# 0xC0000054/pdn-jpegxl

Hardware: AMD Instinct MI355X
Metric: megapixels/sec decode (4K lossy VarDCT) (higher is better)
Workload: dtype f32

## Files before the change

### pdn_jpegxl_amd/csrc/decoder.cc

```cpp
#include <hip/hip_runtime.h>
#include <algorithm>
#include <atomic>
#include <cmath>
#include <cstdarg>
#include <cstdio>
#include <cstdlib>
#include <cstring>
#include <memory>
#include <mutex>
#include <string>
#include <thread>
#include <vector>
#include "../../include/jxlfiletypeio.h"
#include "batch_layout.h"
#include "entropy_plan.h"
#include "host_parse.h"
#include "icc.h"
#include "kernels.h"

namespace jxlhip {

struct HipError : std::runtime_error {
  explicit HipError(const std::string& m) : std::runtime_error(m) {}
};
// ... 64 lines not shown
    std::vector<DevImage> imgs;
    std::vector<int> parse_status;
    std::vector<std::string> parse_msg;
    std::vector<size_t> status_off;
    DevImage* d_imgs = nullptr;
    bool pending = false;
    hipEvent_t lf_done = nullptr, hf_done = nullptr, done = nullptr, uploaded = nullptr;
    std::vector<Tap> taps;
    std::vector<std::string> stage_names;
    std::vector<int> stage_chain;
    std::vector<hipEvent_t> events;
    std::vector<float> stage_ms;
  };
  static constexpr int kSlots = 3;
  static constexpr int kPixelChunk = 32;
  Slot slots[kSlots];
  int cur = 0, last = 0;
  Slot* active = &slots[0];
  hipStream_t stream_lf = nullptr;
  hipStream_t stream_hf = nullptr;
  hipStream_t last_stream = nullptr;
  std::vector<std::string> total_names;
  std::vector<double> total_ms;
  int total_batches = 0;
  std::string sticky_error;
  int sticky_status = 0;
  uint8_t* li_dev = nullptr; uint8_t* li_host = nullptr; size_t li_cap = 0;
  void EnsureLoadImageBuffers(size_t bytes);
  int lane_stride_override = 0;
  int hf_stride_override = 0;
  bool debug_taps = false;
  int band_first_row = 0, band_rows = 0;
  bool no_stream_pairs = false;
  bool no_lf_pipeline = false;
  int alpha_narrow_limit = 32767;
  bool no_direct = false, mod_lanes64 = false;
  bool overlap = true;
  int downscale = 1;

  explicit JxlHipDecoder(int dev);
  ~JxlHipDecoder();
  void EnsureWs(size_t bytes);
  void EnsureBlob(size_t bytes);
  void Mark(const char* name, hipStream_t s, int chain);
  void WaitSlot(Slot& S);
  Slot& Last() { return slots[last]; }
  void Decode(int32_t n_, const uint8_t* const* host_data, const size_t* sizes, const uint8_t* const* dev_data,
              uint8_t* const* dev_out, hipStream_t stream, bool sync, DecoderStatus* statuses, ErrorInfo* err);
  DecoderStatus Finish(DecoderStatus* statuses, ErrorInfo* err);
  void CopyPlaneTap(int stage);
  void PrepassSingle(ParsedFrame& f, const uint8_t* dev_file);
  EntropyPlanOptions PlanOptions() const;
};

JxlHipDecoder::JxlHipDecoder(int dev) {
  if (dev < 0) HIP_OK(hipGetDevice(&dev));
  device = dev;
  HIP_OK(hipSetDevice(device));
  int entropy_cus = 0, pixel_cus = 0;
  if (const char* e = Knob("JXLHIP_ENTROPY_CUS")) entropy_cus = std::min(256, std::max(0, atoi(e)));
  if (const char* e = Knob("JXLHIP_PIXEL_CUS")) pixel_cus = std::min(256, std::max(0, atoi(e)));
  auto masked_stream = [](hipStream_t* s, int first, int count) {
    uint32_t mask[8] = {0, 0, 0, 0, 0, 0, 0, 0};
    for (int i = first; i < first + count; i++) mask[i >> 5] |= 1u << (i & 31);
    HIP_OK(hipExtStreamCreateWithCUMask(s, 8, mask));
  };
// ... 399 lines not shown
  if (any_alpha && !(skip_stages & 4))
    LaunchAlphaAns(d_imgs, B.alpha_tasks, nalpha_t, plan.alpha_stride, plan.alpha.Bytes(), plan.direct_alpha, plan.lean_mod,
                   alpha_narrow, s_hf);
  if (!ds || any_alpha) Mark("alpha_ans", s_hf, 1);
  if (debug_taps && !ds) {
    taps.assign(n, Tap());
    LaunchExpandCoefficients(d_imgs, n, true, B.max_tiles, stream);
    HIP_OK(hipStreamSynchronize(stream));
    CopyPlaneTap(0);
  }
  const bool finish_on_hf = s_hf == stream || debug_taps || !Knob("JXLHIP_ALPHA_FINISH_ON_PIX");
  if (finish_on_hf) {
    if (any_alpha && !(skip_stages & 4)) LaunchAlphaFinish(d_imgs, n, max_groups, alpha_narrow > 0, s_hf);
    if (!ds || any_alpha) Mark("alpha_finish", s_hf, 1);
  }
  if (s_hf != stream) {
    HIP_OK(hipEventRecord(S.hf_done, s_hf));
    HIP_OK(hipStreamWaitEvent(stream, S.hf_done, 0));
  }
  Mark("main_start", stream, 2);
  if (!finish_on_hf) {
    if (any_alpha && !(skip_stages & 4)) LaunchAlphaFinish(d_imgs, n, max_groups, alpha_narrow > 0, stream);
    Mark("alpha_finish", stream, 2);
  }
  hipStream_t s_pix = pix_on_hf ? s_hf : stream;
  if (ds && B.any_vardct) {
    if (any_alpha) LaunchAlphaReduce(d_imgs, n, B.max_ds_cells, s_pix);
    LaunchLfOutput(d_imgs, n, B.max_ds_cells, s_pix);
    Mark("lf_output", s_pix, 2);
  }
  for (int c0 = 0; c0 < (ds ? 0 : n); c0 += pixel_chunk) {
    const int cnt = std::min(pixel_chunk, n - c0);
    if (!(skip_stages & 8))
    LaunchReconTiles(d_imgs + c0, cnt, B.max_tiles, d_basis_all, d_basis_small, d_llf_scale, d_basis_mfma, s_pix);
    Mark("reconstruct", s_pix, 2);
    LaunchExpandCoefficients(d_imgs + c0, cnt, false, B.max_tiles, s_pix);
    LaunchGenericReconstruct(d_imgs + c0, cnt, d_basis_all, d_basis_small, d_llf_scale, s_pix);
    Mark("reconstruct_generic", s_pix, 2);
    if (debug_taps) { HIP_OK(hipStreamSynchronize(s_pix)); CopyPlaneTap(1); }
    if (any_noise && !(early_noise && c0 == 0)) { LaunchNoise(d_imgs + c0, cnt, max_groups, B.max_w, B.max_h, s_pix); Mark("noise", s_pix, 2); }
    if (!(skip_stages & 16))
    LaunchFilterTiles(d_imgs + c0, cnt, B.max_w, B.max_h, B.stage_mask, B.any_unfiltered, B.any_fused, B.any_fused2, s_pix);
    Mark("filters+output", s_pix, 2);
  }
  if (s_pix != stream) {
    HIP_OK(hipEventRecord(S.hf_done, s_pix));
    HIP_OK(hipStreamWaitEvent(stream, S.hf_done, 0));
  }
  if (nmod_t) {
    if (s_lf != stream) { HIP_OK(hipEventRecord(S.lf_done, s_lf)); HIP_OK(hipStreamWaitEvent(stream, S.lf_done, 0)); }
    LaunchModularAns(d_imgs, n, B.mod_tasks, nmod_t, plan.mod.Bytes(), plan.max_mod_groups,
                     plan.max_mod_coded, plan.mod_lanes, plan.mod_rb, plan.mod_wp_lds, plan.direct_mod, stream);
    for (auto& op : B.mod_ops) {
      if (op.kind == 3) LaunchModularPalette(op.a, op.b, op.out, op.nout, op.type, op.rw, op.rh, op.status, stream);
      else LaunchModularOp(op.kind, op.a, op.b, op.c, op.aw, op.ah, op.rw, op.rh, op.type, stream);
    }
    LaunchModularOut(d_imgs, n, B.max_mod_pixels, stream);
    if (ds) LaunchBoxReduce(d_imgs, n, B.max_ds_cells, stream);
    Mark("modular", stream, 2);
  }
  if (!patches.tiles.empty()) {
    LaunchPatches(B.patch_frames, B.patch_tiles, (int)patches.tiles.size(), B.patch_list, B.patch_pos, B.patch_refs, stream);
    Mark("patches", stream, 2);
  }
  if (!comps.empty()) {
    LaunchCompose(B.comp_imgs, B.comp_frames, (int)comps.size(), B.max_segments, stream);
    Mark("compose", stream, 2);
// ... 203 lines not shown
    return DecoderStatus_DecodeError;
  }
}

DecoderStatus jxlhip_finish(JxlHipDecoder* dec, DecoderStatus* statuses, ErrorInfo* err) {
  if (!dec) return DecoderStatus_NullParameter;
  try {
    return dec->Finish(statuses, err);
  } catch (const std::exception& e) {
    SetErr(err, "%s", e.what());
    return DecoderStatus_DecodeError;
  }
}

int32_t jxlhip_set_option(JxlHipDecoder* dec, const char* name, int32_t value) {
  if (!dec || !name) return 0;
  if (!strcmp(name, "debug_taps")) { dec->debug_taps = value != 0; return 1; }
  if (!strcmp(name, "query_pixel_chunk")) return JxlHipDecoder::kPixelChunk;
  if (!strcmp(name, "lane_stride")) { if (value != 0 && !PowerOfTwoUpTo64(value)) return 0; dec->lane_stride_override = value; return 1; }
  if (!strcmp(name, "band_first_row")) { if (value < 0) return 0; dec->band_first_row = value; return 1; }
  if (!strcmp(name, "band_rows")) { if (value < 0) return 0; dec->band_rows = value; return 1; }
  if (!strcmp(name, "no_direct")) { dec->no_direct = value != 0; return 1; }
  if (!strcmp(name, "alpha_narrow_limit")) { if (value < 0 || value > 32767) return 0; dec->alpha_narrow_limit = value; return 1; }
  if (!strcmp(name, "query_alpha_narrow_groups") || !strcmp(name, "query_alpha_redo_groups")) {
    JxlHipDecoder::Slot& S = dec->Last();
    if (S.pending || !S.h_status) return -1;
    const int word = name[12] == 'n' ? kStatusAlphaNarrow : kStatusAlphaRedo;
    int64_t sum = 0;
    for (int i = 0; i < S.n; i++) sum += S.h_status[(size_t)i * 16 + word];
    return (int32_t)std::min<int64_t>(sum, INT32_MAX);
  }
  if (!strcmp(name, "no_stream_pairs")) { dec->no_stream_pairs = value != 0; return 1; }
  if (!strcmp(name, "no_lf_pipeline")) { dec->no_lf_pipeline = value != 0; return 1; }
  if (!strcmp(name, "mod_lanes64")) { dec->mod_lanes64 = value != 0; return 1; }
  if (!strcmp(name, "overlap")) { dec->overlap = value != 0; return 1; }
  if (!strcmp(name, "downscale")) { if (value != 1 && value != 8) return 0; dec->downscale = value; return 1; }
  return 0;
}

size_t jxlhip_read_plane(JxlHipDecoder* dec, int32_t index, const char* name, int32_t channel, void* dst, size_t capacity) {
  if (!dec || !name) return 0;
  JxlHipDecoder::Slot& S = dec->Last();
  if (index < 0 || index >= S.n || S.pending) return 0;
  if (S.parse_status[index] != DecoderStatus_Ok) return 0;
  const DevImage& d = S.imgs[index];
  std::string nm(name);
  const size_t cells = (size_t)d.w8 * d.h8, pix = (size_t)d.wp * d.hp;
  const void* src = nullptr;
  size_t bytes = 0;
  bool host = false;
  const int c = std::min(2, std::max(0, channel));
  if (nm == "lf") { src = d.lf_final[c]; bytes = cells * 4; }
  else if (nm == "lf_quant") { src = d.lfq[c]; bytes = cells * 4; }
  else if (nm == "cellinfo") { src = d.cellinfo; bytes = cells * 4; }
  else if (nm == "raw_quant") { src = d.rawq; bytes = cells * 2; }
  else if (nm == "sharpness") { src = d.sharp; bytes = cells; }
  else if (nm == "ytox") { src = d.ytox; bytes = (size_t)d.wt * d.ht; }
  else if (nm == "ytob") { src = d.ytob; bytes = (size_t)d.wt * d.ht; }
  else if (nm == "alpha") { src = d.alpha; bytes = (size_t)d.w * d.h; }
  else if (nm == "inv_sigma") { src = d.inv_sigma; bytes = cells * 4; }
  else if (dec->debug_taps && (size_t)index < S.taps.size()) {
    host = true;
    if (nm == "qcoef") { src = S.taps[index].qcoef[c].data(); bytes = S.taps[index].qcoef[c].size(); }
    else if (nm == "xyb_idct") { src = S.taps[index].xyb_idct[c].data(); bytes = S.taps[index].xyb_idct[c].size(); }
    else if (nm == "xyb_filtered") { src = S.taps[index].xyb_filtered[c].data(); bytes = S.taps[index].xyb_filtered[c].size(); }
    else if (nm == "noise_rnd") { src = S.taps[index].noise_rnd[c].data(); bytes = S.taps[index].noise_rnd[c].size(); }
// ... 230 lines not shown
```

### pdn_jpegxl_amd/csrc/kernels.h

```cpp
#pragma once
#include <hip/hip_runtime.h>
#include "dev_types.h"

namespace jxlhip {

void LaunchLfAns(const DevImage* imgs, const SectionTask* tasks, int ntasks, int slots, size_t lds_bytes, int scalar_rows, bool lean, hipStream_t s);
void LaunchLfFinish(const DevImage* imgs, const SectionTask* tasks, int ntasks, bool pipeline, hipStream_t s);
void LaunchHfBlockList(const DevImage* imgs, int nimg, int max_groups, hipStream_t s);
void LaunchHfDecode(const DevImage* imgs, const SectionTask* tasks, int nwg, int threads, int lane_stride, size_t lds_bytes, size_t lane_bytes,
                    hipStream_t s);
void LaunchAlphaAns(const DevImage* imgs, const SectionTask* tasks, int nwg, int lane_stride, size_t lds_bytes, int scalar_rows, bool lean, int narrow_limit,
                    hipStream_t s);
void LaunchAlphaFinish(const DevImage* imgs, int nimg, int max_groups, bool narrow, hipStream_t s);
void LaunchModularAns(const DevImage* imgs, int nimg, const SectionTask* tasks, int ntasks, size_t lds_bytes, int max_sections, int max_coded,
                      int lanes, int rb_width, int wp_lds, int scalar_rows, hipStream_t s);
void LaunchModularOp(int kind, int32_t* a, int32_t* b, int32_t* c, int aw, int ah, int rw, int rh, int type, hipStream_t s);
void LaunchModularPalette(const int32_t* palette, const int32_t* index, int32_t* const* out, int nout, int nb_colors, int w, int h, uint32_t* status,
                          hipStream_t s);
void LaunchModularOut(const DevImage* imgs, int nimg, size_t max_pixels, hipStream_t s);
void LaunchOrient(const uint8_t* src, uint8_t* dst, int w, int h, int px_bytes, int orientation, hipStream_t s);
void LaunchLfPixelStages(const DevImage* imgs, int nimg, size_t max_cells, hipStream_t s);
void LaunchExpandCoefficients(const DevImage* imgs, int nimg, bool all_tiles, int max_tiles, hipStream_t s);
void LaunchGenericReconstruct(const DevImage* imgs, int nimg, const float* basis_all, const float* basis_small,
                              const float* llf_scale, hipStream_t s);
void LaunchReconTiles(const DevImage* imgs, int nimg, int max_tiles, const float* basis_all, const float* basis_small,
                      const float* llf_scale, const float* basis_mfma, hipStream_t s);
void LaunchFilterTiles(const DevImage* imgs, int nimg, int max_w, int max_h, int stage_mask, bool any_unfiltered,
                       int any_fused, int any_fused2, hipStream_t s);

void LaunchLfOutput(const DevImage* imgs, int nimg, size_t max_cells, hipStream_t s);
void LaunchAlphaReduce(const DevImage* imgs, int nimg, size_t max_cells, hipStream_t s);
void LaunchBoxReduce(const DevImage* imgs, int nimg, size_t max_cells, hipStream_t s);

void LaunchNoise(const DevImage* imgs, int nimg, int max_groups, int max_w, int max_h, hipStream_t s);

void LaunchCompose(const ComposeImage* imgs, const ComposeFrame* frames, int nimg, int max_segments, hipStream_t s);
void LaunchPatches(const PatchFrame* frames, const PatchTile* tiles, int ntiles, const int32_t* list, const PatchPos* pos, const PatchRef* refs,
                   hipStream_t s);

void LaunchStatusToHost(const uint32_t* src, uint32_t* dst_pinned, int nwords, hipStream_t s);
#ifdef JXLHIP_EXPERIMENTS
void LaunchInterference(int kind, int wg_per_cu, int lds_kb, float ms, float* scratch, size_t scratch_bytes, hipStream_t s);
#endif

}
```

### pdn_jpegxl_amd/csrc/tile_kernels.hip

```cpp
#include <hip/hip_runtime.h>
#include <cstdlib>
#include "dev_types.h"
#include "dev_util.h"
#include "kernels.h"

namespace jxlhip {

#ifndef JXLHIP_PRIO_PIXEL
#define JXLHIP_PRIO_PIXEL 0
#endif
#if JXLHIP_PRIO_PIXEL
#define JXL_PIXEL_PRIO() __builtin_amdgcn_s_setprio(JXLHIP_PRIO_PIXEL)
#else
#define JXL_PIXEL_PRIO() ((void)0)
#endif

namespace {

constexpr int kTS = 64;
constexpr int kLP = 65;

__device__ const uint8_t t_quant_table[kNumStrategies] = {0, 1, 2, 3, 4, 5, 6, 6, 7, 7, 8, 8, 9, 9, 10, 10, 10, 10, 11, 12, 12, 13, 14, 14, 15, 16, 16};

__device__ __forceinline__ bool Special(uint32_t s) { return (s >= 1 && s <= 3) || (s >= 12 && s <= 17); }
typedef float __attribute__((ext_vector_type(4))) F4;
template <int N>
__device__ __forceinline__ F4 MfmaChain(const float* pa, int sa, const float* pb, int sb) {
  float a[N / 4], b[N / 4];
#pragma unroll
  for (int k = 0; k < N / 4; k++) { a[k] = pa[k * sa]; b[k] = pb[k * sb]; }
  F4 acc = {0.f, 0.f, 0.f, 0.f};
#pragma unroll
  for (int k = 0; k < N / 4; k++) acc = __builtin_amdgcn_mfma_f32_16x16x4f32(a[k], b[k], acc, 0, 0, 0);
  return acc;
}
template <bool kTableIsA>
__device__ __forceinline__ F4 MfmaChain32L(const float4* t_lo, const float4* t_hi, int pair, const float* po, int so) {
  const float4 v0 = t_lo[pair], v1 = t_hi[pair];
  const float t[8] = {v0.x, v0.y, v0.z, v0.w, v1.x, v1.y, v1.z, v1.w};
  float o[8];
#pragma unroll
  for (int k = 0; k < 8; k++) o[k] = po[k * so];
  F4 acc = {0.f, 0.f, 0.f, 0.f};
#pragma unroll
  for (int k = 0; k < 8; k++)
    acc = kTableIsA ? __builtin_amdgcn_mfma_f32_16x16x4f32(t[k], o[k], acc, 0, 0, 0) : __builtin_amdgcn_mfma_f32_16x16x4f32(o[k], t[k], acc, 0, 0, 0);
  return acc;
}
template <bool kTableIsA>
__device__ __forceinline__ F4 MfmaChain64L(const float4* t64, int pair, const float* po, int so) {
  float t[16], o[16];
#pragma unroll
  for (int j = 0; j < 4; j++) {
    const float4 v = t64[j * 256 + pair];
    t[4 * j] = v.x; t[4 * j + 1] = v.y; t[4 * j + 2] = v.z; t[4 * j + 3] = v.w;
  }
#pragma unroll
  for (int k = 0; k < 16; k++) o[k] = po[k * so];
  F4 acc = {0.f, 0.f, 0.f, 0.f};
#pragma unroll
  for (int k = 0; k < 16; k++)
    acc = kTableIsA ? __builtin_amdgcn_mfma_f32_16x16x4f32(t[k], o[k], acc, 0, 0, 0) : __builtin_amdgcn_mfma_f32_16x16x4f32(o[k], t[k], acc, 0, 0, 0);
  return acc;
}
__device__ __forceinline__ bool MfmaRows(uint32_t tl, uint32_t tr) {
  return (tl >> 31) && (tr >> 31) && ((tl >> 21) & 7) >= 1 && ((tl >> 21) & 7) == ((tr >> 21) & 7) && ((tl >> 13) & 31) == ((tr >> 13) & 31);
}
__device__ __forceinline__ bool MfmaCols(uint32_t tl, uint32_t bl) {
  return (tl >> 31) && (bl >> 31) && ((tl >> 18) & 7) >= 1 && ((tl >> 18) & 7) == ((bl >> 18) & 7) && ((tl >> 8) & 31) == ((bl >> 8) & 31);
}

__device__ __forceinline__ float SrgbOetfT(float v) {
  const float lin = 12.92f * v;
  const float cur = 1.055f * __builtin_amdgcn_exp2f(__builtin_amdgcn_logf(v) * (1.0f / 2.4f)) - 0.055f;
  return v <= 0.0031308f ? lin : cur;
}
__device__ __forceinline__ float SrgbOetf255T(float v) {
  const float lin = (12.92f * 255.0f) * v;
  const float cur = (1.055f * 255.0f) * __builtin_amdgcn_exp2f(__builtin_amdgcn_logf(v) * (1.0f / 2.4f)) - (0.055f * 255.0f);
  return v <= 0.0031308f ? lin : cur;
}
__device__ __forceinline__ float PowT(float a, float e) { return __builtin_amdgcn_exp2f(__builtin_amdgcn_logf(a) * e); }
__device__ __forceinline__ float EncodeTransferT(int kind, float v, float pq_scale, const float* lut = nullptr) {
  if (kind == 0) return v;
  if (kind == 5) {
    const float t = __builtin_sqrtf(fminf(fmaxf(v, 0.f), 1.f)) * 4095.0f;
    const int i = min((int)t, 4094);
    return lut[i] + (lut[i + 1] - lut[i]) * (t - (float)i);
  }
  const float a = fabsf(v);
  float r;
  if (kind == 1) r = a <= 0.0031308f ? 12.92f * a : 1.055f * PowT(a, 1.0f / 2.4f) - 0.055f;
  else if (kind == 2) r = a < 0.018f ? 4.5f * a : 1.099f * PowT(a, 0.45f) - 0.099f;
  else {
    const float xp = a > 0.f ? PowT(a * pq_scale, 0.1593017578125f) : 0.f;
    r = a > 0.f ? PowT((0.8359375f + 18.8515625f * xp) / (1.0f + 18.6875f * xp), 78.84375f) : 0.f;
  }
// ... 103 lines not shown
  }
  WritePixelA(im, x, y, X, Y, B, a);
}
__device__ __forceinline__ void WritePixel(const DevImage& im, int x, int y, float X, float Y, float B) {
  const uint32_t a = im.has_alpha ? LoadAlpha(im, (size_t)y * im.w + x) : 0u;
  if (im.has_noise) { WritePixelGeneral(im, x, y, X, Y, B, a); return; }
  WritePixelA(im, x, y, X, Y, B, a);
}

}

#define JXL_IDCT_STEP(Bp, v0, v1)                                                                  \
  {                                                                                                \
    const float4 b0 = *(const float4*)(Bp);                                                        \
    const float4 b1 = *(const float4*)((Bp) + 4);                                                  \
    a0[0] += v0 * b0.x; a0[1] += v0 * b0.y; a0[2] += v0 * b0.z; a0[3] += v0 * b0.w;                \
    a0[4] += v0 * b1.x; a0[5] += v0 * b1.y; a0[6] += v0 * b1.z; a0[7] += v0 * b1.w;                \
    a1[0] += v1 * b0.x; a1[1] += v1 * b0.y; a1[2] += v1 * b0.z; a1[3] += v1 * b0.w;                \
    a1[4] += v1 * b1.x; a1[5] += v1 * b1.y; a1[6] += v1 * b1.z; a1[7] += v1 * b1.w;                \
  }

__device__ __forceinline__ float DequantBias(int32_t v, float qb, float qb3) {
  if (v == 0) return 0.f;
  if (v == 1) return qb;
  if (v == -1) return -qb;
  const float f = (float)v;
  return f - qb3 * __builtin_amdgcn_rcpf(f);
}
typedef int __attribute__((ext_vector_type(4))) I4v;

constexpr int kTileF = kTS * kLP;

__global__ __launch_bounds__(768, 6) void recon_tile_kernel(const DevImage* __restrict__ imgs, const float* basis_all, const float* basis_small,
                                                             const float* llf_scale, const float* basis_mfma) {
  JXL_PIXEL_PRIO();
  extern __shared__ __align__(16) uint8_t smem_raw[];
  float* cfc3 = (float*)smem_raw;
  float* B816 = cfc3 + 3 * kTileF;
  float* cscale = B816 + 320;
  uint32_t* ci = (uint32_t*)(cscale + 64);
  uint32_t* cmeta = ci + 64;
  uint32_t* cnq = cmeta + 64;
  uint32_t* cpre = cnq + 64;
  uint32_t* cstart = cpre + 3 * 64;
  uint32_t* ctot = cstart + 3 * 64;
  const U32x2** csc = (const U32x2**)(ctot + 4);
  float4* t32_lo = (float4*)(csc + 64);
  float4* t32_hi = t32_lo + 128;
  float4* t64 = t32_hi + 128;
  const DevImage& im = imgs[blockIdx.y];
  const int tile = blockIdx.x;
  if (tile >= im.wt * im.ht) return;
  const int tid = threadIdx.x;
  const int tx = tile % im.wt, ty = tile / im.wt;
  if (ty < im.dec_gy0 * 4 || ty >= im.dec_gy1 * 4) return;
  const int wave = tid >> 6, lane = tid & 63, team = wave >> 2, tw = wave & 3;
  const int c = team == 0 ? 1 : (team == 1 ? 0 : 2);
  const int wp = im.wp, hp = im.hp;
  {
    float4* z = (float4*)cfc3;
    for (int i = tid; i < 3 * kTileF / 4; i += 768) z[i] = make_float4(0.f, 0.f, 0.f, 0.f);
  }
  int bad = 0, has64 = 0;
  if (tid < 64) {
    const int cx = tx * 8 + (tid & 7), cy = ty * 8 + (tid >> 3);
    const bool inside = cx < im.w8 && cy < im.h8;
    const size_t cell_g = (size_t)min(cy, im.h8 - 1) * im.w8 + min(cx, im.w8 - 1);
    const size_t ncells = (size_t)im.w8 * im.h8;
    const uint32_t info_g = im.cellinfo[cell_g];
    const uint32_t rq_g = im.rawq[cell_g];
    U32x2 blk[3];
    blk[0] = im.cblk[ncells + cell_g]; blk[1] = im.cblk[cell_g]; blk[2] = im.cblk[2 * ncells + cell_g];
    const uint32_t info = inside ? info_g : 0u;
    const uint32_t rqv = inside ? rq_g : 1u;
    const int ix = (info >> 8) & 31, iy = (info >> 13) & 31, lcx = (info >> 18) & 7, lcy = (info >> 21) & 7;
    if (inside) {
      if (!(info >> 31)) bad = 1;
      else {
        const int ox = (tid & 7) - ix, oy = (tid >> 3) - iy;
        bad = ox < 0 || oy < 0 || ox + (1 << lcx) > 8 || oy + (1 << lcy) > 8 || Special(info & 0xFF) ||
              (ox & ((1 << lcx) - 1)) != 0 || (oy & ((1 << lcy) - 1)) != 0;
      }
    }
    const bool valid = (info >> 31) && !bad;
    has64 = valid && (lcx == 3 || lcy == 3);
    {
      const uint64_t any = __ballot(has64);
      if (tid == 0) ctot[3] = any != 0;
    }
    const uint32_t q = t_quant_table[valid ? (info & 0xFF) : 0];
    const uint32_t rq_origin = (uint32_t)__shfl((int)rqv, valid ? tid - iy * 8 - ix : tid);
    const uint32_t lng = 3 + max(lcx, lcy);
    const bool transposed = lcy >= lcx;
    ci[tid] = info;
    cscale[tid] = im.inv_global_scale / (float)rq_origin;
    cmeta[tid] = lng | (transposed ? 16u : 0u);
    cnq[tid] = im.dq_n[q];
    csc[tid] = im.scan[q];
    const bool origin = valid && ix == 0 && iy == 0;
    uint32_t cnt[3], sum[3];
#pragma unroll
    for (int t = 0; t < 3; t++) {
      cnt[t] = origin ? blk[t].y : 0u;
      if (cnt[t] > 65536u || blk[t].x > kGroupEntriesCap - cnt[t]) cnt[t] = 0;
      sum[t] = cnt[t];
    }
#pragma unroll
    for (int d = 1; d < 64; d <<= 1) {
#pragma unroll
      for (int t = 0; t < 3; t++) {
        const uint32_t a = (uint32_t)__shfl_up((int)sum[t], d);
        if (tid >= d) sum[t] += a;
      }
    }
#pragma unroll
    for (int t = 0; t < 3; t++) {
      cpre[t * 64 + tid] = sum[t] - cnt[t];
      cstart[t * 64 + tid] = blk[t].x;
      if (tid == 63) ctot[t] = sum[t];
    }
  } else if (tid < 64 + 320) {
    B816[tid - 64] = basis_all[tid - 64];
  } else if (tid < 64 + 320 + 256) {
    const int i = tid - (64 + 320);
    const float4 v = ((const float4*)basis_mfma)[i];
    if (i & 1) t32_hi[i >> 1] = v; else t32_lo[i >> 1] = v;
  }
  if (im.num_passes > 1) bad = 1;
  if (__syncthreads_or(bad)) {
    if (tid == 0) im.tile_list[atomicAdd(&im.status[1], 1u)] = (uint32_t)tile;
    return;
  }
  if (ctot[3]) {
    for (int i = tid; i < 1024; i += 768) t64[(i & 3) * 256 + (i >> 2)] = ((const float4*)(basis_mfma + 1024))[i];
  }
  const float* const Bl = basis_all;
  float* const cfc = cfc3 + team * kTileF;
  if (tw == 0) {
    const int cxg = tx * 8 + (lane & 7), cyg = ty * 8 + (lane >> 3);
    const bool inside = cxg < im.w8 && cyg < im.h8;
    const float lf_g = im.lf_final[c][(size_t)min(cyg, im.h8 - 1) * im.w8 + min(cxg, im.w8 - 1)];
    const float lfv = inside ? lf_g : 0.f;
    const uint32_t info = ci[lane];
    const bool valid = info >> 31;
    const int ix = (info >> 8) & 31, iy = (info >> 13) & 31, lcx = (info >> 18) & 7, lcy = (info >> 21) & 7;
    const int cx = 1 << lcx, cy = 1 << lcy;
    const int ox = (lane & 7) - ix, oy = (lane >> 3) - iy;
    const float* Bx = basis_small + (cx * cx - 1) / 3 + ix * cx;
    const float* By = basis_small + (cy * cy - 1) / 3 + iy * cy;
    float bx[8], byv[8];
#pragma unroll
// ... 11 lines not shown
      const float v = __shfl(row, ((oy + k) * 8 + (lane & 7)) & 63);
      if (valid && k < cy) acc += v * byv[k];
    }
    if (valid) atomicAdd(&cfc[(oy * 8 + iy) * kLP + ox * 8 + ix], acc * sc);
  }
  {
    const size_t tile_cfl = (size_t)ty * im.wt + tx;
    const float cfl_x = im.base_x + (float)im.ytox[tile_cfl] * im.inv_color_factor;
    const float cfl_b = im.base_b + (float)im.ytob[tile_cfl] * im.inv_color_factor;
    const uint32_t* entries = im.centries + (size_t)((ty >> 2) * im.xg + (tx >> 2) - im.centries_g0) * kGroupEntriesCap;
    const uint32_t t0 = ctot[0], t01 = t0 + ctot[1], total = t01 + ctot[2];
    const float qb3 = im.qbias[3];
    for (uint32_t e = (uint32_t)tid; e < total; e += 768) {
      const uint32_t t = (e >= t0) + (e >= t01);
      const uint32_t el = e - (t == 0 ? 0u : (t == 1 ? t0 : t01));
      const uint32_t* pre = cpre + t * 64;
      uint32_t j = 0;
#pragma unroll
      for (int step = 32; step; step >>= 1) if (pre[j + step] <= el) j += step;
      const uint32_t ent = entries[cstart[t * 64 + j] + (el - pre[j])];
      const uint32_t k = ent & 0xFFFFu, nq = cnq[j];
      if (k >= nq) continue;
      const int chan = t == 0 ? 1 : (t == 1 ? 0 : 2);
      const U32x2 se = csc[j][(size_t)chan * nq + k];
      const uint32_t meta = cmeta[j];
      const uint32_t lng = meta & 15, p = se.x;
      const uint32_t r = p >> lng, cc = p & ((1u << lng) - 1);
      const uint32_t ky = (meta & 16) ? cc : r, kx = (meta & 16) ? r : cc;
      if (ky >= 64 || kx >= 64) continue;
      const int32_t v = (int32_t)ent >> 16;
      const float dm = t == 0 ? 1.0f : (t == 1 ? im.x_dm : im.b_dm);
      const float o = DequantBias(v, im.qbias[chan], qb3) * (cscale[j] * dm) * __uint_as_float(se.y);
      const uint32_t at = ((j >> 3) * 8 + ky) * kLP + (j & 7) * 8 + kx;
      atomicAdd(&cfc3[t * kTileF + at], o);
      if (t == 0) {
        if (cfl_x != 0.f) atomicAdd(&cfc3[kTileF + at], o * cfl_x);
        if (cfl_b != 0.f) atomicAdd(&cfc3[2 * kTileF + at], o * cfl_b);
      }
    }
  }
  __syncthreads();
  const int l16 = tid & 15, lq = lane >> 4;
  {
    F4 acc[4];
    bool m[4];
    const int x0 = tw * 16;
#pragma unroll
    for (int rb = 0; rb < 4; rb++) {
      const uint32_t inf = ci[rb * 16 + tw * 2];
      m[rb] = MfmaRows(inf, ci[rb * 16 + tw * 2 + 1]);
      if (m[rb]) {
        const int iy = (inf >> 13) & 31, lcy = (inf >> 21) & 7, R = 8 << lcy;
        const float* cp = cfc + ((rb * 2 - iy) * 8 + lq) * kLP + x0 + l16;
        if (R == 16) acc[rb] = MfmaChain<16>(B816 + 64 + lq * 16 + iy * 8 + l16, 64, cp, 4 * kLP);
        else if (R == 32) acc[rb] = MfmaChain32L<true>(t32_lo, t32_hi, (iy * 8 + l16) * 4 + lq, cp, 4 * kLP);
        else acc[rb] = MfmaChain64L<true>(t64, (iy * 8 + l16) * 4 + lq, cp, 4 * kLP);
      }
    }
    const int x = x0 + (lane & 7) * 2, cr = lane >> 3;
    const uint32_t info = ci[cr * 8 + (x >> 3)];
    const bool valu = (info >> 31) && !MfmaRows(ci[(cr >> 1) * 16 + (x >> 4) * 2], ci[(cr >> 1) * 16 + (x >> 4) * 2 + 1]);
    float a0[8] = {0, 0, 0, 0, 0, 0, 0, 0}, a1[8] = {0, 0, 0, 0, 0, 0, 0, 0};
    if (valu) {
      const int iy = (info >> 13) & 31, lcy = (info >> 21) & 7;
      const int R = 8 << lcy;
      const float* in = cfc + (cr - iy) * 8 * kLP + x;
      if (R == 8) {
#pragma unroll 2
        for (int k = 0; k < 8; k++) { const float v0 = in[k * kLP], v1 = in[k * kLP + 1]; JXL_IDCT_STEP(B816 + k * 8, v0, v1) }
      } else if (R == 16) {
        const float* B = B816 + 64 + iy * 8;
#pragma unroll 2
        for (int k = 0; k < 16; k++) { const float v0 = in[k * kLP], v1 = in[k * kLP + 1]; JXL_IDCT_STEP(B + k * 16, v0, v1) }
      } else {
        const float* B = Bl + (R * R - 64) / 3 + iy * 8;
        for (int k = 0; k < R; k++) { const float v0 = in[k * kLP], v1 = in[k * kLP + 1]; JXL_IDCT_STEP(B + k * R, v0, v1) }
      }
    }
    __builtin_amdgcn_fence(__ATOMIC_RELEASE, "wavefront");
    __builtin_amdgcn_wave_barrier();
#pragma unroll
    for (int rb = 0; rb < 4; rb++)
      if (m[rb]) {
        float* o = cfc + (rb * 16 + 4 * lq) * kLP + x0 + l16;
        o[0] = acc[rb].x; o[kLP] = acc[rb].y; o[2 * kLP] = acc[rb].z; o[3 * kLP] = acc[rb].w;
      }
    if (valu) {
#pragma unroll
      for (int j = 0; j < 8; j++) { cfc[(cr * 8 + j) * kLP + x] = a0[j]; cfc[(cr * 8 + j) * kLP + x + 1] = a1[j]; }
    }
  }
  __syncthreads();
  {
    F4 acc[4];
    bool m[4];
    const int y0 = tw * 16;
#pragma unroll
    for (int cs = 0; cs < 4; cs++) {
      const uint32_t inf = ci[tw * 16 + cs * 2];
      m[cs] = MfmaCols(inf, ci[tw * 16 + 8 + cs * 2]);
      if (m[cs]) {
        const int ix = (inf >> 8) & 31, lcx = (inf >> 18) & 7, C = 8 << lcx;
        const float* ap = cfc + (y0 + l16) * kLP + (cs * 2 - ix) * 8 + lq;
        if (C == 16) acc[cs] = MfmaChain<16>(ap, 4, B816 + 64 + lq * 16 + ix * 8 + l16, 64);
        else if (C == 32) acc[cs] = MfmaChain32L<false>(t32_lo, t32_hi, (ix * 8 + l16) * 4 + lq, ap, 4);
        else acc[cs] = MfmaChain64L<false>(t64, (ix * 8 + l16) * 4 + lq, ap, 4);
      }
    }
    const int y = y0 + (lane & 7) * 2, cc = lane >> 3;
    const uint32_t info = ci[(y >> 3) * 8 + cc];
    const bool valu = (info >> 31) && !MfmaCols(ci[(y >> 4) * 16 + (cc >> 1) * 2], ci[(y >> 4) * 16 + 8 + (cc >> 1) * 2]);
    float a0[8] = {0, 0, 0, 0, 0, 0, 0, 0}, a1[8] = {0, 0, 0, 0, 0, 0, 0, 0};
    if (valu) {
      const int ix = (info >> 8) & 31, lcx = (info >> 18) & 7;
      const int C = 8 << lcx;
      const float* in = cfc + y * kLP + (cc - ix) * 8;
      if (C == 8) {
#pragma unroll 2
        for (int k = 0; k < 8; k++) { const float v0 = in[k], v1 = in[k + kLP]; JXL_IDCT_STEP(B816 + k * 8, v0, v1) }
      } else if (C == 16) {
        const float* B = B816 + 64 + ix * 8;
#pragma unroll 2
        for (int k = 0; k < 16; k++) { const float v0 = in[k], v1 = in[k + kLP]; JXL_IDCT_STEP(B + k * 16, v0, v1) }
      } else {
        const float* B = Bl + (C * C - 64) / 3 + ix * 8;
        for (int k = 0; k < C; k++) { const float v0 = in[k], v1 = in[k + kLP]; JXL_IDCT_STEP(B + k * C, v0, v1) }
      }
    }
    __builtin_amdgcn_fence(__ATOMIC_RELEASE, "wavefront");
    __builtin_amdgcn_wave_barrier();
#pragma unroll
    for (int cs = 0; cs < 4; cs++)
      if (m[cs]) {
        float* o = cfc + (y0 + 4 * lq) * kLP + cs * 16 + l16;
        o[0] = acc[cs].x; o[kLP] = acc[cs].y; o[2 * kLP] = acc[cs].z; o[3 * kLP] = acc[cs].w;
      }
    if (valu) {
#pragma unroll
      for (int j = 0; j < 8; j++) { cfc[y * kLP + cc * 8 + j] = a0[j]; cfc[(y + 1) * kLP + cc * 8 + j] = a1[j]; }
    }
    __builtin_amdgcn_fence(__ATOMIC_ACQ_REL, "wavefront");
    __builtin_amdgcn_wave_barrier();
    float* dst = im.xyb[c];
    const int x4 = l16 * 4;
    const int gx = tx * kTS + x4;
#pragma unroll
    for (int it = 0; it < 4; it++) {
      const int yl = y0 + lq + 4 * it;
      const int gy = ty * kTS + yl;
      const float* r = cfc + yl * kLP + x4;
      const float4 o = make_float4(r[0], r[1], r[2], r[3]);
      if (gx < wp && gy < hp) *(float4*)(dst + (size_t)gy * wp + gx) = o;
    }
  }
}

template <int kStage>
__global__ __launch_bounds__(256) void filter_tile_kernel(const DevImage* __restrict__ imgs) {
// ... 660 lines not shown
  if (!im.ds || im.is_modular) return;
  const size_t n = (size_t)im.ds_w * im.ds_h;
  const float* __restrict__ pX = im.lf_final[0];
  const float* __restrict__ pY = im.lf_final[1];
  const float* __restrict__ pB = im.lf_final[2];
  const size_t gid = (size_t)blockIdx.x * blockDim.x + threadIdx.x, stride = (size_t)gridDim.x * blockDim.x;
  const bool quads = PlainOutput(im) && im.ds_orient == 1 && im.ncolor == 3 && ((uintptr_t)im.out & 15) == 0;
  if (!quads) {
    for (size_t i = gid; i < n; i += stride) LfOutputPixel(im, i, pX[i], pY[i], pB[i]);
    return;
  }
  const size_t nq = n >> 2;
  for (size_t q = gid; q < nq; q += stride) {
    const float4 X = ((const float4*)pX)[q], Y = ((const float4*)pY)[q], B = ((const float4*)pB)[q];
    const uint32_t a = im.has_alpha ? ((const uint32_t*)im.ds_alpha)[q] : 0u;
    const uint32_t p0 = PixelToRgba8(im, X.x, Y.x, B.x, a & 0xFF), p1 = PixelToRgba8(im, X.y, Y.y, B.y, (a >> 8) & 0xFF);
    const uint32_t p2 = PixelToRgba8(im, X.z, Y.z, B.z, (a >> 16) & 0xFF), p3 = PixelToRgba8(im, X.w, Y.w, B.w, a >> 24);
    if (im.nch_out == 4) ((uint4*)im.out)[q] = make_uint4(p0, p1, p2, p3);
    else ((uint3*)im.out)[q] = make_uint3((p0 & 0xFFFFFFu) | (p1 << 24), ((p1 >> 8) & 0xFFFFu) | (p2 << 16), ((p2 >> 16) & 0xFFu) | (p3 << 8));
  }
  if (blockIdx.x == 0 && threadIdx.x < (n & 3)) {
    const size_t i = 4 * nq + threadIdx.x;
    LfOutputPixel(im, i, pX[i], pY[i], pB[i]);
  }
}

void LaunchLfOutput(const DevImage* imgs, int nimg, size_t max_cells, hipStream_t s) {
  if (nimg <= 0) return;
  const size_t b = std::min<size_t>((max_cells + 255) / 256, 2048);
  hipLaunchKernelGGL(lf_output_kernel, dim3((unsigned)std::max<size_t>(1, b), nimg), dim3(256), 0, s, imgs);
}

void LaunchReconTiles(const DevImage* imgs, int nimg, int max_tiles, const float* basis_all, const float* basis_small,
                      const float* llf_scale, const float* basis_mfma, hipStream_t s) {
  const size_t lds = (size_t)(3 * kTileF + 320 + 64 * 4 + 64 * 6 + 4 + 128 + 1024 + 4096) * 4;
  static bool raised = false;
  if (!raised) { (void)hipFuncSetAttribute((const void*)recon_tile_kernel, hipFuncAttributeMaxDynamicSharedMemorySize, (int)lds); raised = true; }
  hipLaunchKernelGGL(recon_tile_kernel, dim3(max_tiles, nimg), dim3(768), lds, s, imgs, basis_all, basis_small, llf_scale, basis_mfma);
}

void LaunchFilterTiles(const DevImage* imgs, int nimg, int max_w, int max_h, int stage_mask, bool any_unfiltered,
                       int any_fused, int any_fused2, hipStream_t s) {
  const int tiles = ((max_w + 63) / 64) * ((max_h + 31) / 32);
  dim3 g(tiles, nimg);
  if (stage_mask & 1) hipLaunchKernelGGL(filter_tile_kernel<0>, g, dim3(256), 0, s, imgs);
  if (stage_mask & 2) hipLaunchKernelGGL(filter_tile_kernel<1>, g, dim3(256), 0, s, imgs);
  if (any_fused) {
    const int groups = ((max_w + kStripOut - 1) / kStripOut) * ((max_h + 2 + kSegRows - 1) / kSegRows);
    const int pair_groups = ((max_w + kPairOut - 1) / kPairOut) * ((max_h + 2 + kSegRows - 1) / kSegRows);
    if (any_fused & 1) hipLaunchKernelGGL(filter_stream_pairs_kernel, dim3((pair_groups + kGroupsPerWg - 1) / kGroupsPerWg, nimg), dim3(256), 0, s, imgs);
    if (any_fused & 2) hipLaunchKernelGGL(filter_stream_kernel, dim3((groups + kGroupsPerWg - 1) / kGroupsPerWg, nimg), dim3(256), 0, s, imgs);
    const int pair2_groups = ((max_w + kPair2Out - 1) / kPair2Out) * ((max_h + kSegRows - 1) / kSegRows);
    if (any_fused2 & 1) hipLaunchKernelGGL(filter_stream2_pairs_kernel, dim3((pair2_groups + kGroupsPerWg - 1) / kGroupsPerWg, nimg), dim3(256), 0, s, imgs);
    if (any_fused2 & 2) hipLaunchKernelGGL(filter_stream2_kernel, dim3((groups + kGroupsPerWg - 1) / kGroupsPerWg, nimg), dim3(256), 0, s, imgs);
  }
  if (stage_mask & 4) hipLaunchKernelGGL(filter_tile_kernel<2>, g, dim3(256), 0, s, imgs);
  if (stage_mask & 8) hipLaunchKernelGGL(filter_tile_kernel<3>, g, dim3(256), 0, s, imgs);
  if (any_unfiltered) {
    size_t work = (size_t)max_w * max_h;
    size_t b = std::min<size_t>((work + 255) / 256, 8192);
    hipLaunchKernelGGL(out_only_kernel, dim3((unsigned)b, nimg), dim3(256), 0, s, imgs);
  }
}

}
```

Measured before the change: 33750.

## Skip zero coefficient extents in MFMA IDCT chains via per-block extent bitmasks

```diff
diff --git a/pdn_jpegxl_amd/csrc/decoder.cc b/pdn_jpegxl_amd/csrc/decoder.cc
--- a/pdn_jpegxl_amd/csrc/decoder.cc
+++ b/pdn_jpegxl_amd/csrc/decoder.cc
@@ -120,6 +120,7 @@
   bool debug_taps = false;
   int band_first_row = 0, band_rows = 0;
   bool no_stream_pairs = false;
+  bool recon_dense = false;
   bool no_lf_pipeline = false;
   int alpha_narrow_limit = 32767;
   bool no_direct = false, mod_lanes64 = false;
@@ -585,7 +586,7 @@
   for (int c0 = 0; c0 < (ds ? 0 : n); c0 += pixel_chunk) {
     const int cnt = std::min(pixel_chunk, n - c0);
     if (!(skip_stages & 8))
-    LaunchReconTiles(d_imgs + c0, cnt, B.max_tiles, d_basis_all, d_basis_small, d_llf_scale, d_basis_mfma, s_pix);
+    LaunchReconTiles(d_imgs + c0, cnt, B.max_tiles, d_basis_all, d_basis_small, d_llf_scale, d_basis_mfma, recon_dense, s_pix);
     Mark("reconstruct", s_pix, 2);
     LaunchExpandCoefficients(d_imgs + c0, cnt, false, B.max_tiles, s_pix);
     LaunchGenericReconstruct(d_imgs + c0, cnt, d_basis_all, d_basis_small, d_llf_scale, s_pix);
@@ -855,6 +856,7 @@
   }
   if (!strcmp(name, "no_stream_pairs")) { dec->no_stream_pairs = value != 0; return 1; }
   if (!strcmp(name, "no_lf_pipeline")) { dec->no_lf_pipeline = value != 0; return 1; }
+  if (!strcmp(name, "recon_dense")) { dec->recon_dense = value != 0; return 1; }
   if (!strcmp(name, "mod_lanes64")) { dec->mod_lanes64 = value != 0; return 1; }
   if (!strcmp(name, "overlap")) { dec->overlap = value != 0; return 1; }
   if (!strcmp(name, "downscale")) { if (value != 1 && value != 8) return 0; dec->downscale = value; return 1; }
diff --git a/pdn_jpegxl_amd/csrc/kernels.h b/pdn_jpegxl_amd/csrc/kernels.h
--- a/pdn_jpegxl_amd/csrc/kernels.h
+++ b/pdn_jpegxl_amd/csrc/kernels.h
@@ -24,7 +24,7 @@
 void LaunchGenericReconstruct(const DevImage* imgs, int nimg, const float* basis_all, const float* basis_small,
                               const float* llf_scale, hipStream_t s);
 void LaunchReconTiles(const DevImage* imgs, int nimg, int max_tiles, const float* basis_all, const float* basis_small,
-                      const float* llf_scale, const float* basis_mfma, hipStream_t s);
+                      const float* llf_scale, const float* basis_mfma, bool dense, hipStream_t s);
 void LaunchFilterTiles(const DevImage* imgs, int nimg, int max_w, int max_h, int stage_mask, bool any_unfiltered,
                        int any_fused, int any_fused2, hipStream_t s);
 
diff --git a/pdn_jpegxl_amd/csrc/tile_kernels.hip b/pdn_jpegxl_amd/csrc/tile_kernels.hip
--- a/pdn_jpegxl_amd/csrc/tile_kernels.hip
+++ b/pdn_jpegxl_amd/csrc/tile_kernels.hip
@@ -24,45 +24,53 @@
 
 __device__ __forceinline__ bool Special(uint32_t s) { return (s >= 1 && s <= 3) || (s >= 12 && s <= 17); }
 typedef float __attribute__((ext_vector_type(4))) F4;
+template <int K, int N, typename F>
+__device__ __forceinline__ void WhileBelow(int nk, F&& f) {
+  if constexpr (K < N) {
+    if (K < nk) { f(K); WhileBelow<K + 1, N>(nk, f); }
+  }
+}
 template <int N>
-__device__ __forceinline__ F4 MfmaChain(const float* pa, int sa, const float* pb, int sb) {
+__device__ __forceinline__ F4 MfmaChain(const float* pa, int sa, const float* pb, int sb, int nk) {
   float a[N / 4], b[N / 4];
-#pragma unroll
-  for (int k = 0; k < N / 4; k++) { a[k] = pa[k * sa]; b[k] = pb[k * sb]; }
+  WhileBelow<0, N / 4>(nk, [&](int k) { a[k] = pa[k * sa]; b[k] = pb[k * sb]; });
   F4 acc = {0.f, 0.f, 0.f, 0.f};
-#pragma unroll
-  for (int k = 0; k < N / 4; k++) acc = __builtin_amdgcn_mfma_f32_16x16x4f32(a[k], b[k], acc, 0, 0, 0);
+  WhileBelow<0, N / 4>(nk, [&](int k) { acc = __builtin_amdgcn_mfma_f32_16x16x4f32(a[k], b[k], acc, 0, 0, 0); });
   return acc;
 }
 template <bool kTableIsA>
-__device__ __forceinline__ F4 MfmaChain32L(const float4* t_lo, const float4* t_hi, int pair, const float* po, int so) {
-  const float4 v0 = t_lo[pair], v1 = t_hi[pair];
-  const float t[8] = {v0.x, v0.y, v0.z, v0.w, v1.x, v1.y, v1.z, v1.w};
-  float o[8];
-#pragma unroll
-  for (int k = 0; k < 8; k++) o[k] = po[k * so];
+__device__ __forceinline__ F4 MfmaChain32L(const float4* t_lo, const float4* t_hi, int pair, const float* po, int so, int nk) {
+  float t[8], o[8];
+  WhileBelow<0, 2>((nk + 3) >> 2, [&](int j) {
+    const float4 v = (j ? t_hi : t_lo)[pair];
+    t[4 * j] = v.x; t[4 * j + 1] = v.y; t[4 * j + 2] = v.z; t[4 * j + 3] = v.w;
+  });
+  WhileBelow<0, 8>(nk, [&](int k) { o[k] = po[k * so]; });
   F4 acc = {0.f, 0.f, 0.f, 0.f};
-#pragma unroll
-  for (int k = 0; k < 8; k++)
+  WhileBelow<0, 8>(nk, [&](int k) {
     acc = kTableIsA ? __builtin_amdgcn_mfma_f32_16x16x4f32(t[k], o[k], acc, 0, 0, 0) : __builtin_amdgcn_mfma_f32_16x16x4f32(o[k], t[k], acc, 0, 0, 0);
+  });
   return acc;
 }
 template <bool kTableIsA>
-__device__ __forceinline__ F4 MfmaChain64L(const float4* t64, int pair, const float* po, int so) {
-  float t[16], o[16];
-#pragma unroll
-  for (int j = 0; j < 4; j++) {
-    const float4 v = t64[j * 256 + pair];
-    t[4 * j] = v.x; t[4 * j + 1] = v.y; t[4 * j + 2] = v.z; t[4 * j + 3] = v.w;
-  }
-#pragma unroll
-  for (int k = 0; k < 16; k++) o[k] = po[k * so];
+__device__ __forceinline__ F4 MfmaChain64L(const float4* t64, int pair, const float* po, int so, int nk) {
   F4 acc = {0.f, 0.f, 0.f, 0.f};
-#pragma unroll
-  for (int k = 0; k < 16; k++)
-    acc = kTableIsA ? __builtin_amdgcn_mfma_f32_16x16x4f32(t[k], o[k], acc, 0, 0, 0) : __builtin_amdgcn_mfma_f32_16x16x4f32(o[k], t[k], acc, 0, 0, 0);
+  WhileBelow<0, 2>((nk + 7) >> 3, [&](int h) {
+    float t[8], o[8];
+    const int nh = nk - 8 * h;
+    WhileBelow<0, 2>((nh + 3) >> 2, [&](int j) {
+      const float4 v = t64[(2 * h + j) * 256 + pair];
+      t[4 * j] = v.x; t[4 * j + 1] = v.y; t[4 * j + 2] = v.z; t[4 * j + 3] = v.w;
+    });
+    WhileBelow<0, 8>(nh, [&](int k) { o[k] = po[(8 * h + k) * so]; });
+    WhileBelow<0, 8>(nh, [&](int k) {
+      acc = kTableIsA ? __builtin_amdgcn_mfma_f32_16x16x4f32(t[k], o[k], acc, 0, 0, 0) : __builtin_amdgcn_mfma_f32_16x16x4f32(o[k], t[k], acc, 0, 0, 0);
+    });
+  });
   return acc;
 }
+__device__ __forceinline__ uint32_t ExtentBits(uint32_t ky, uint32_t kx) { return (1u << (ky >> 2)) | (0x10000u << (kx >> 2)); }
+__device__ __forceinline__ int StepsOf(uint32_t set16) { return 32 - __clz((int)(set16 & 0xFFFFu)); }
 __device__ __forceinline__ bool MfmaRows(uint32_t tl, uint32_t tr) {
   return (tl >> 31) && (tr >> 31) && ((tl >> 21) & 7) >= 1 && ((tl >> 21) & 7) == ((tr >> 21) & 7) && ((tl >> 13) & 31) == ((tr >> 13) & 31);
 }
@@ -232,7 +240,7 @@
 constexpr int kTileF = kTS * kLP;
 
 __global__ __launch_bounds__(768, 6) void recon_tile_kernel(const DevImage* __restrict__ imgs, const float* basis_all, const float* basis_small,
-                                                             const float* llf_scale, const float* basis_mfma) {
+                                                             const float* llf_scale, const float* basis_mfma, int dense) {
   JXL_PIXEL_PRIO();
   extern __shared__ __align__(16) uint8_t smem_raw[];
   float* cfc3 = (float*)smem_raw;
@@ -248,6 +256,7 @@
   float4* t32_lo = (float4*)(csc + 64);
   float4* t32_hi = t32_lo + 128;
   float4* t64 = t32_hi + 128;
+  uint32_t* cext = (uint32_t*)(t64 + 1024);
   const DevImage& im = imgs[blockIdx.y];
   const int tile = blockIdx.x;
   if (tile >= im.wt * im.ht) return;
@@ -292,12 +301,13 @@
     const uint32_t rq_origin = (uint32_t)__shfl((int)rqv, valid ? tid - iy * 8 - ix : tid);
     const uint32_t lng = 3 + max(lcx, lcy);
     const bool transposed = lcy >= lcx;
+    const bool origin = valid && ix == 0 && iy == 0;
     ci[tid] = info;
     cscale[tid] = im.inv_global_scale / (float)rq_origin;
     cmeta[tid] = lng | (transposed ? 16u : 0u);
     cnq[tid] = im.dq_n[q];
     csc[tid] = im.scan[q];
-    const bool origin = valid && ix == 0 && iy == 0;
+    const uint32_t llf_bits = origin ? ExtentBits((1u << lcy) - 1, (1u << lcx) - 1) : 0u;
     uint32_t cnt[3], sum[3];
 #pragma unroll
     for (int t = 0; t < 3; t++) {
@@ -317,6 +327,7 @@
     for (int t = 0; t < 3; t++) {
       cpre[t * 64 + tid] = sum[t] - cnt[t];
       cstart[t * 64 + tid] = blk[t].x;
+      cext[t * 64 + tid] = llf_bits;
       if (tid == 63) ctot[t] = sum[t];
     }
   } else if (tid < 64 + 320) {
@@ -394,29 +405,43 @@
       const float dm = t == 0 ? 1.0f : (t == 1 ? im.x_dm : im.b_dm);
       const float o = DequantBias(v, im.qbias[chan], qb3) * (cscale[j] * dm) * __uint_as_float(se.y);
       const uint32_t at = ((j >> 3) * 8 + ky) * kLP + (j & 7) * 8 + kx;
+      const uint32_t bits = ExtentBits(ky, kx);
       atomicAdd(&cfc3[t * kTileF + at], o);
+      atomicOr(&cext[t * 64 + j], bits);
       if (t == 0) {
-        if (cfl_x != 0.f) atomicAdd(&cfc3[kTileF + at], o * cfl_x);
-        if (cfl_b != 0.f) atomicAdd(&cfc3[2 * kTileF + at], o * cfl_b);
+        if (cfl_x != 0.f) { atomicAdd(&cfc3[kTileF + at], o * cfl_x); atomicOr(&cext[64 + j], bits); }
+        if (cfl_b != 0.f) { atomicAdd(&cfc3[2 * kTileF + at], o * cfl_b); atomicOr(&cext[128 + j], bits); }
       }
     }
   }
   __syncthreads();
   const int l16 = tid & 15, lq = lane >> 4;
+  const uint32_t* const ext = cext + (__builtin_amdgcn_readfirstlane(wave) >> 2) * 64;
   {
     F4 acc[4];
     bool m[4];
     const int x0 = tw * 16;
+    uint32_t plans = 0;
+    {
+      const int sb = lane & 3;
+      const uint32_t inf = ci[sb * 16 + tw * 2], inf_r = ci[sb * 16 + tw * 2 + 1];
+      const bool mfma = MfmaRows(inf, inf_r);
+      const int iy = (inf >> 13) & 31, lcy = (inf >> 21) & 7;
+      const int ix_l = (inf >> 8) & 31, ix_r = (inf_r >> 8) & 31;
+      const uint32_t e_l = ext[mfma ? (sb * 2 - iy) * 8 + tw * 2 - ix_l : 0], e_r = ext[mfma ? (sb * 2 - iy) * 8 + tw * 2 + 1 - ix_r : 0];
+      const bool live = ((e_l >> (16 + 2 * ix_l)) | (e_r >> (16 + 2 * ix_r))) != 0;
+      if (mfma) plans = (uint32_t)min(2 << lcy, StepsOf(e_l | e_r)) | (iy << 5) | (lcy << 10) | (live ? 1u << 13 : 0u) | (1u << 14);
+    }
 #pragma unroll
     for (int rb = 0; rb < 4; rb++) {
-      const uint32_t inf = ci[rb * 16 + tw * 2];
-      m[rb] = MfmaRows(inf, ci[rb * 16 + tw * 2 + 1]);
+      const uint32_t plan = __builtin_amdgcn_readlane(plans, rb);
+      m[rb] = (plan >> 13) == 3 || (dense && (plan >> 14));
       if (m[rb]) {
-        const int iy = (inf >> 13) & 31, lcy = (inf >> 21) & 7, R = 8 << lcy;
+        const int iy = (plan >> 5) & 31, R = 8 << ((plan >> 10) & 7), nk = dense ? R >> 2 : plan & 31;
         const float* cp = cfc + ((rb * 2 - iy) * 8 + lq) * kLP + x0 + l16;
-        if (R == 16) acc[rb] = MfmaChain<16>(B816 + 64 + lq * 16 + iy * 8 + l16, 64, cp, 4 * kLP);
-        else if (R == 32) acc[rb] = MfmaChain32L<true>(t32_lo, t32_hi, (iy * 8 + l16) * 4 + lq, cp, 4 * kLP);
-        else acc[rb] = MfmaChain64L<true>(t64, (iy * 8 + l16) * 4 + lq, cp, 4 * kLP);
+        if (R == 16) acc[rb] = MfmaChain<16>(B816 + 64 + lq * 16 + iy * 8 + l16, 64, cp, 4 * kLP, nk);
+        else if (R == 32) acc[rb] = MfmaChain32L<true>(t32_lo, t32_hi, (iy * 8 + l16) * 4 + lq, cp, 4 * kLP, nk);
+        else acc[rb] = MfmaChain64L<true>(t64, (iy * 8 + l16) * 4 + lq, cp, 4 * kLP, nk);
       }
     }
     const int x = x0 + (lane & 7) * 2, cr = lane >> 3;
@@ -432,10 +457,11 @@
         for (int k = 0; k < 8; k++) { const float v0 = in[k * kLP], v1 = in[k * kLP + 1]; JXL_IDCT_STEP(B816 + k * 8, v0, v1) }
       } else if (R == 16) {
         const float* B = B816 + 64 + iy * 8;
-#pragma unroll 2
+#pragma unroll 1
         for (int k = 0; k < 16; k++) { const float v0 = in[k * kLP], v1 = in[k * kLP + 1]; JXL_IDCT_STEP(B + k * 16, v0, v1) }
       } else {
         const float* B = Bl + (R * R - 64) / 3 + iy * 8;
+#pragma unroll 1
         for (int k = 0; k < R; k++) { const float v0 = in[k * kLP], v1 = in[k * kLP + 1]; JXL_IDCT_STEP(B + k * R, v0, v1) }
       }
     }
@@ -457,16 +483,26 @@
     F4 acc[4];
     bool m[4];
     const int y0 = tw * 16;
+    uint32_t plans = 0;
+    {
+      const int sb = lane & 3;
+      const uint32_t inf = ci[tw * 16 + sb * 2], inf_b = ci[tw * 16 + 8 + sb * 2];
+      const bool mfma = MfmaCols(inf, inf_b);
+      const int ix = (inf >> 8) & 31, lcx = (inf >> 18) & 7;
+      const int iy_t = (inf >> 13) & 31, iy_b = (inf_b >> 13) & 31;
+      const uint32_t e_t = ext[mfma ? (tw * 2 - iy_t) * 8 + sb * 2 - ix : 0], e_b = ext[mfma ? (tw * 2 + 1 - iy_b) * 8 + sb * 2 - ix : 0];
+      if (mfma) plans = (uint32_t)min(2 << lcx, StepsOf((e_t | e_b) >> 16)) | (ix << 5) | (lcx << 10) | (1u << 14);
+    }
 #pragma unroll
     for (int cs = 0; cs < 4; cs++) {
-      const uint32_t inf = ci[tw * 16 + cs * 2];
-      m[cs] = MfmaCols(inf, ci[tw * 16 + 8 + cs * 2]);
+      const uint32_t plan = __builtin_amdgcn_readlane(plans, cs);
+      m[cs] = (plan >> 14) != 0;
       if (m[cs]) {
-        const int ix = (inf >> 8) & 31, lcx = (inf >> 18) & 7, C = 8 << lcx;
+        const int ix = (plan >> 5) & 31, C = 8 << ((plan >> 10) & 7), nk = dense ? C >> 2 : plan & 31;
         const float* ap = cfc + (y0 + l16) * kLP + (cs * 2 - ix) * 8 + lq;
-        if (C == 16) acc[cs] = MfmaChain<16>(ap, 4, B816 + 64 + lq * 16 + ix * 8 + l16, 64);
-        else if (C == 32) acc[cs] = MfmaChain32L<false>(t32_lo, t32_hi, (ix * 8 + l16) * 4 + lq, ap, 4);
-        else acc[cs] = MfmaChain64L<false>(t64, (ix * 8 + l16) * 4 + lq, ap, 4);
+        if (C == 16) acc[cs] = MfmaChain<16>(ap, 4, B816 + 64 + lq * 16 + ix * 8 + l16, 64, nk);
+        else if (C == 32) acc[cs] = MfmaChain32L<false>(t32_lo, t32_hi, (ix * 8 + l16) * 4 + lq, ap, 4, nk);
+        else acc[cs] = MfmaChain64L<false>(t64, (ix * 8 + l16) * 4 + lq, ap, 4, nk);
       }
     }
     const int y = y0 + (lane & 7) * 2, cc = lane >> 3;
@@ -486,6 +522,7 @@
         for (int k = 0; k < 16; k++) { const float v0 = in[k], v1 = in[k + kLP]; JXL_IDCT_STEP(B + k * 16, v0, v1) }
       } else {
         const float* B = Bl + (C * C - 64) / 3 + ix * 8;
+#pragma unroll 1
         for (int k = 0; k < C; k++) { const float v0 = in[k], v1 = in[k + kLP]; JXL_IDCT_STEP(B + k * C, v0, v1) }
       }
     }
@@ -1212,11 +1249,12 @@
 }
 
 void LaunchReconTiles(const DevImage* imgs, int nimg, int max_tiles, const float* basis_all, const float* basis_small,
-                      const float* llf_scale, const float* basis_mfma, hipStream_t s) {
-  const size_t lds = (size_t)(3 * kTileF + 320 + 64 * 4 + 64 * 6 + 4 + 128 + 1024 + 4096) * 4;
+                      const float* llf_scale, const float* basis_mfma, bool dense, hipStream_t s) {
+  const size_t lds = (size_t)(3 * kTileF + 320 + 64 * 4 + 64 * 6 + 4 + 128 + 1024 + 4096 + 3 * 64) * 4;
+  static_assert((3 * kTileF + 320 + 64 * 4 + 64 * 6 + 4 + 128 + 1024 + 4096 + 3 * 64) * 4 <= 80 * 1024, "two workgroups of recon_tile_kernel must fit a CU's LDS");
   static bool raised = false;
   if (!raised) { (void)hipFuncSetAttribute((const void*)recon_tile_kernel, hipFuncAttributeMaxDynamicSharedMemorySize, (int)lds); raised = true; }
-  hipLaunchKernelGGL(recon_tile_kernel, dim3(max_tiles, nimg), dim3(768), lds, s, imgs, basis_all, basis_small, llf_scale, basis_mfma);
+  hipLaunchKernelGGL(recon_tile_kernel, dim3(max_tiles, nimg), dim3(768), lds, s, imgs, basis_all, basis_small, llf_scale, basis_mfma, dense ? 1 : 0);
 }
 
 void LaunchFilterTiles(const DevImage* imgs, int nimg, int max_w, int max_h, int stage_mask, bool any_unfiltered,
```

Result: no change. 33660 (-0.3%).
